# showlab/EgoVLP

Measured on NVIDIA H100. Metric: clips/sec, 16-frame TimeSformer-B + DistilBERT + EgoNCE training step, higher is better.
Workload: dtype bf16

## Files before the change

egovlp_b200/csrc/attention.cu:

```cuda
#include <stdlib.h>

#include "common.cuh"
#include "egovlp_b200.h"

namespace egovlp {

bool space_attn_wgmma_supported(int N);
int space_attn_fwd_wgmma(const void* qkv, void* out, float* lse, float* cls_part, int B, int T, int N, int H,
                         cudaStream_t st);

namespace {

constexpr int HD = 64;
constexpr int ROW_BYTES = 128;
constexpr float LOG2E = 1.4426950408889634f;

struct Geom {
  int B, H, T, N, S, D;
  int mode;
  int PG;
  int G;
  int NP;
  int NPAD;
  int gsize;
};

__device__ __forceinline__ int row_token(const Geom& G, int g, int r) {
  if (r == G.NP) return 0;
  if (r > G.NP) return -1;
  if (G.mode == 1) return 1 + g * G.N + r;
  const int j = r / G.T, f = r - j * G.T, n = g * G.PG + j;
  return n < G.N ? 1 + f * G.N + n : -1;
}

template <int RT>
__device__ __forceinline__ int row_token_x(const Geom& G, int g, int r, int sh) {
  if (RT == 0) return row_token(G, g, r);
  if (r == G.NP) return 0;
  if (r > G.NP) return -1;
  if (RT == 1) return 1 + g * G.N + r;
  const int n = g * G.PG + (r >> sh);
  return n < G.N ? 1 + (r & ((1 << sh) - 1)) * G.N + n : -1;
}

struct Smem {
  uint32_t q, k, v, dout;
  short* gid;
  float* lse;
  float* delta;
  uint32_t stage;
  uint32_t bar;
};

__device__ __forceinline__ bool pair_valid(int gq, int gk, bool first_group) {
  if (gq >= 0) return gk == gq || gk == -2;
  if (gq == -2) return gk >= 0 || (gk == -2 && first_group);
  return false;
}

__device__ __forceinline__ void tile_window(const Geom& G, int r0, int& lo, int& hi) {
  if (r0 <= G.NP && G.NP < r0 + 16) { lo = 0; hi = G.NP; return; }
  if (r0 > G.NP) { lo = 0; hi = 0; return; }
  lo = (r0 / G.gsize) * G.gsize;
  hi = min(G.NP, ((r0 + 15) / G.gsize + 1) * G.gsize);
}
__device__ __forceinline__ bool span_active(const Geom& G, int lo, int hi, int c0, int width) {
  return (c0 < hi && c0 + width > lo) || (c0 <= G.NP && G.NP < c0 + width);
}

template <int RT = 0>
__device__ __forceinline__ void store_rows_bf16(const float (&acc)[8][4], float s0, float s1, uint32_t stage,
                                                uint8_t* stage_gen, bf16* dst, long long ld, int col0, const Geom& G,
                                                int b, int g, int r0, int lane, bool skip_cls, int sh = 0) {
  const int gq = lane >> 2, t = lane & 3;
#pragma unroll
  for (int j = 0; j < 8; ++j) {
    const uint32_t lo = pack_bf16x2(acc[j][0] * s0, acc[j][1] * s0), hi = pack_bf16x2(acc[j][2] * s1, acc[j][3] * s1);
    asm volatile("st.shared.b32 [%0], %1;" ::"r"(sw_addr(stage, gq, j) + t * 4), "r"(lo));
    asm volatile("st.shared.b32 [%0], %1;" ::"r"(sw_addr(stage, gq + 8, j) + t * 4), "r"(hi));
  }
  __syncwarp();
#pragma unroll
  for (int p = 0; p < 4; ++p) {
    const int rr = p * 4 + (lane >> 3), c = lane & 7;
    const int tok = row_token_x<RT>(G, g, r0 + rr, sh);
    if (tok > 0 || (tok == 0 && !skip_cls)) {
      const uint4 v = *reinterpret_cast<const uint4*>(stage_gen + (sw_addr(stage, rr, c) - stage));
      *reinterpret_cast<uint4*>(dst + ((long long)b * G.S + tok) * ld + col0 + c * 8) = v;
    }
  }
  __syncwarp();
}
// ... 1012 lines not shown


}
}

using namespace egovlp;

extern "C" long long egovlp_divided_attn_workspace_floats(int B, int T, int N, int H, int mode) {
  Geom G;
  if (make_geom(G, B, T, N, H, mode)) return -1;
  return (long long)B * H * G.G * 4 * 66;
}

extern "C" int egovlp_divided_attn_fwd(const void* qkv, void* out, float* lse, float* cls_part, int B, int T, int N,
                                       int H, int mode, void* stream) {
  EGOVLP_CHECK_ARG(qkv && out && lse && cls_part, "divided_attn_fwd: null pointer");
  EGOVLP_CHECK_ARG(B > 0 && T > 0 && N > 0 && H > 0 && (mode == 0 || mode == 1), "divided_attn_fwd: bad shape");
  Geom G;
  if (make_geom(G, B, T, N, H, mode)) { set_last_error("divided_attn: unsupported geometry T=%d N=%d", T, N); return EGOVLP_ERR_UNSUPPORTED; }
  CUtensorMap tm;
  int rc = make_group_tmap(&tm, qkv, G, 3 * H);
  if (rc) return rc;
  cudaStream_t st = reinterpret_cast<cudaStream_t>(stream);
  const bf16* q = reinterpret_cast<const bf16*>(qkv);
  bf16* o = reinterpret_cast<bf16*>(out);
  const int grid = B * H * G.G;
#define LAUNCH_FWD(KERN, W, ...)                                                                              \
  do {                                                                                                        \
    const size_t smem = attn_smem_bytes(G, false, W, generic || mode == 1);                                   \
    EGOVLP_CHECK_CUDA(cudaFuncSetAttribute(KERN, cudaFuncAttributeMaxDynamicSharedMemorySize, (int)smem));    \
    KERN<<<grid, W * 32, smem, st>>>(tm, q, o, lse, cls_part, G, ##__VA_ARGS__);                              \
  } while (0)
  const bool generic = force_generic() || (mode == 0 && !time_fast_ok(G));
  if (!generic && mode == 1 && space_attn_wgmma_supported(N)) {
    rc = space_attn_fwd_wgmma(qkv, out, lse, cls_part, B, T, N, H, st);
    if (rc) return rc;
  } else if (generic) {
    if (G.NPAD > 128) LAUNCH_FWD((divided_attn_fwd_kernel<7, 2>), 7);
    else LAUNCH_FWD((divided_attn_fwd_kernel<4, 3>), 4);
  } else if (mode == 1) {
    if (G.NPAD > 128) LAUNCH_FWD((fast_attn_fwd_kernel<false, 7, 2>), 7, 0);
    else LAUNCH_FWD((fast_attn_fwd_kernel<false, 4, 3>), 4, 0);
  } else {
    LAUNCH_FWD((fast_attn_fwd_kernel<true, 4, 4>), 4, time_shift(G));
  }
#undef LAUNCH_FWD
  EGOVLP_CHECK_LAUNCH();
  const int BH = B * H;
  const int parts = (!generic && mode == 0) ? 4 : 1;
  cls_merge_kernel<<<(BH + 3) / 4, 128, 0, st>>>(cls_part, o, lse, BH, H, G.G * parts, G.S, G.D);
  EGOVLP_CHECK_LAUNCH();
  return EGOVLP_OK;
}

extern "C" int egovlp_divided_attn_bwd(const void* qkv, const void* out, const void* dout, const float* lse,
                                       void* dqkv, float* dcls_ws, int B, int T, int N, int H, int mode,
                                       float q_scale, void* stream) {
  EGOVLP_CHECK_ARG(qkv && out && dout && lse && dqkv && dcls_ws, "divided_attn_bwd: null pointer");
  EGOVLP_CHECK_ARG(B > 0 && T > 0 && N > 0 && H > 0 && (mode == 0 || mode == 1), "divided_attn_bwd: bad shape");
  Geom G;
  if (make_geom(G, B, T, N, H, mode)) { set_last_error("divided_attn: unsupported geometry T=%d N=%d", T, N); return EGOVLP_ERR_UNSUPPORTED; }
  CUtensorMap tmq, tmd;
  int rc = make_group_tmap(&tmq, qkv, G, 3 * H);
  if (rc) return rc;
  rc = make_group_tmap(&tmd, dout, G, H);
  if (rc) return rc;
  cudaStream_t st = reinterpret_cast<cudaStream_t>(stream);
  EGOVLP_CHECK_CUDA(cudaMemsetAsync(dcls_ws, 0, (size_t)B * H * 3 * HD * sizeof(float), st));
  const bf16* q = reinterpret_cast<const bf16*>(qkv);
  const bf16* o = reinterpret_cast<const bf16*>(out);
  const bf16* d_o = reinterpret_cast<const bf16*>(dout);
  bf16* dq = reinterpret_cast<bf16*>(dqkv);
  const int grid = B * H * G.G;
#define LAUNCH_BWD(KERN, W, ...)                                                                              \
  do {                                                                                                        \
    const size_t smem = attn_smem_bytes(G, true, W);                                                          \
    EGOVLP_CHECK_CUDA(cudaFuncSetAttribute(KERN, cudaFuncAttributeMaxDynamicSharedMemorySize, (int)smem));    \
    KERN<<<grid, W * 32, smem, st>>>(tmq, tmd, q, o, d_o, lse, dq, dcls_ws, q_scale, G, ##__VA_ARGS__);       \
  } while (0)
  const bool generic = force_generic() || (mode == 0 && !time_fast_ok(G));
  if (generic) {
    if (G.NPAD > 128) LAUNCH_BWD((divided_attn_bwd_kernel<7, 2>), 7);
    else LAUNCH_BWD((divided_attn_bwd_kernel<4, 3>), 4);
  } else if (mode == 1) {
    if (G.NPAD > 128) LAUNCH_BWD((fast_attn_bwd_kernel<false, 7, 2>), 7, 0);
    else LAUNCH_BWD((fast_attn_bwd_kernel<false, 4, 3>), 4, 0);
  } else {
    const char* we = getenv("EGOVLP_ATTN_TIME_BWD_WARPS");
    const bool w8 = we && we[0] == '8';
    if (w8) LAUNCH_BWD((fast_attn_bwd_kernel<true, 8, 2>), 8, time_shift(G));
    else LAUNCH_BWD((fast_attn_bwd_kernel<true, 4, 3>), 4, time_shift(G));
  }
#undef LAUNCH_BWD
  EGOVLP_CHECK_LAUNCH();
  const int n = B * H * 3 * HD;
  cls_grad_finalize_kernel<<<(n + 255) / 256, 256, 0, st>>>(dcls_ws, reinterpret_cast<bf16*>(dqkv), B, H, G.S, G.D, q_scale);
  EGOVLP_CHECK_LAUNCH();
  return EGOVLP_OK;
}
```

egovlp_b200/csrc/attention_wgmma.cu:

```cuda
#include <stdlib.h>

#include "common.cuh"
#include "egovlp_b200.h"

namespace egovlp {
namespace {

constexpr int HD = 64;
constexpr int ROWB = 128;
constexpr int QROWS = 256;
constexpr int KROWS = 208;
constexpr int Q_BYTES = QROWS * ROWB, KV_BYTES = KROWS * ROWB;
constexpr int SMEM_BYTES = Q_BYTES + 2 * KV_BYTES + 1024  + 64 ;
constexpr float LOG2E = 1.4426950408889634f;

struct SpaceGeom {
  int H, T, N, S, D;
};

__device__ __forceinline__ void wgmma_m64n208k16_ss(float (&d)[104], uint64_t adesc, uint64_t bdesc, int scale_d) {
  asm volatile(
      "{\n\t.reg .pred p;\n\t"
      "setp.ne.b32 p, %106, 0;\n\t"
      "wgmma.mma_async.sync.aligned.m64n208k16.f32.bf16.bf16 "
      "{%0,%1,%2,%3,%4,%5,%6,%7,%8,%9,%10,%11,%12,%13,%14,%15,%16,%17,%18,%19,%20,%21,%22,%23,%24,%25,%26,%27,%28,%29,%30,%31,"
      "%32,%33,%34,%35,%36,%37,%38,%39,%40,%41,%42,%43,%44,%45,%46,%47,%48,%49,%50,%51,%52,%53,%54,%55,%56,%57,%58,%59,%60,%61,%62,%63,"
      "%64,%65,%66,%67,%68,%69,%70,%71,%72,%73,%74,%75,%76,%77,%78,%79,%80,%81,%82,%83,%84,%85,%86,%87,%88,%89,%90,%91,%92,%93,%94,%95,"
      "%96,%97,%98,%99,%100,%101,%102,%103}, "
      "%104, %105, p, 1, 1, 0, 0;\n\t}"
      : "+f"(d[0]), "+f"(d[1]), "+f"(d[2]), "+f"(d[3]), "+f"(d[4]), "+f"(d[5]), "+f"(d[6]), "+f"(d[7]),
        "+f"(d[8]), "+f"(d[9]), "+f"(d[10]), "+f"(d[11]), "+f"(d[12]), "+f"(d[13]), "+f"(d[14]), "+f"(d[15]),
        "+f"(d[16]), "+f"(d[17]), "+f"(d[18]), "+f"(d[19]), "+f"(d[20]), "+f"(d[21]), "+f"(d[22]), "+f"(d[23]),
        "+f"(d[24]), "+f"(d[25]), "+f"(d[26]), "+f"(d[27]), "+f"(d[28]), "+f"(d[29]), "+f"(d[30]), "+f"(d[31]),
        "+f"(d[32]), "+f"(d[33]), "+f"(d[34]), "+f"(d[35]), "+f"(d[36]), "+f"(d[37]), "+f"(d[38]), "+f"(d[39]),
        "+f"(d[40]), "+f"(d[41]), "+f"(d[42]), "+f"(d[43]), "+f"(d[44]), "+f"(d[45]), "+f"(d[46]), "+f"(d[47]),
        "+f"(d[48]), "+f"(d[49]), "+f"(d[50]), "+f"(d[51]), "+f"(d[52]), "+f"(d[53]), "+f"(d[54]), "+f"(d[55]),
        "+f"(d[56]), "+f"(d[57]), "+f"(d[58]), "+f"(d[59]), "+f"(d[60]), "+f"(d[61]), "+f"(d[62]), "+f"(d[63]),
        "+f"(d[64]), "+f"(d[65]), "+f"(d[66]), "+f"(d[67]), "+f"(d[68]), "+f"(d[69]), "+f"(d[70]), "+f"(d[71]),
        "+f"(d[72]), "+f"(d[73]), "+f"(d[74]), "+f"(d[75]), "+f"(d[76]), "+f"(d[77]), "+f"(d[78]), "+f"(d[79]),
        "+f"(d[80]), "+f"(d[81]), "+f"(d[82]), "+f"(d[83]), "+f"(d[84]), "+f"(d[85]), "+f"(d[86]), "+f"(d[87]),
        "+f"(d[88]), "+f"(d[89]), "+f"(d[90]), "+f"(d[91]), "+f"(d[92]), "+f"(d[93]), "+f"(d[94]), "+f"(d[95]),
        "+f"(d[96]), "+f"(d[97]), "+f"(d[98]), "+f"(d[99]), "+f"(d[100]), "+f"(d[101]), "+f"(d[102]), "+f"(d[103])
      : "l"(adesc), "l"(bdesc), "r"(scale_d));
}
__device__ __forceinline__ void wgmma_m64n64k16_rs(float (&d)[32], uint32_t a0, uint32_t a1, uint32_t a2, uint32_t a3,
                                                  uint64_t bdesc, int scale_d) {
  asm volatile(
      "{\n\t.reg .pred p;\n\t"
      "setp.ne.b32 p, %37, 0;\n\t"
      "wgmma.mma_async.sync.aligned.m64n64k16.f32.bf16.bf16 "
      "{%0,%1,%2,%3,%4,%5,%6,%7,%8,%9,%10,%11,%12,%13,%14,%15,%16,%17,%18,%19,%20,%21,%22,%23,%24,%25,%26,%27,%28,%29,%30,%31}, "
      "{%32, %33, %34, %35}, %36, p, 1, 1, 1;\n\t}"
      : "+f"(d[0]), "+f"(d[1]), "+f"(d[2]), "+f"(d[3]), "+f"(d[4]), "+f"(d[5]), "+f"(d[6]), "+f"(d[7]),
        "+f"(d[8]), "+f"(d[9]), "+f"(d[10]), "+f"(d[11]), "+f"(d[12]), "+f"(d[13]), "+f"(d[14]), "+f"(d[15]),
        "+f"(d[16]), "+f"(d[17]), "+f"(d[18]), "+f"(d[19]), "+f"(d[20]), "+f"(d[21]), "+f"(d[22]), "+f"(d[23]),
        "+f"(d[24]), "+f"(d[25]), "+f"(d[26]), "+f"(d[27]), "+f"(d[28]), "+f"(d[29]), "+f"(d[30]), "+f"(d[31])
      : "r"(a0), "r"(a1), "r"(a2), "r"(a3), "l"(bdesc), "r"(scale_d));
}

__global__ void __launch_bounds__(256, 1)
space_attn_fwd_wgmma_kernel(const __grid_constant__ CUtensorMap tm_rows, const __grid_constant__ CUtensorMap tm_cls,
                            bf16* __restrict__ out, float* __restrict__ lse_out, float* __restrict__ cls_part, SpaceGeom G) {
  extern __shared__ uint8_t smem_raw[];
  const uint32_t base = (smem_u32(smem_raw) + 1023u) & ~1023u;
  uint8_t* gen = smem_raw + (base - smem_u32(smem_raw));
  const uint32_t sQ = base, sK = base + Q_BYTES, sV = sK + KV_BYTES, bar = sV + KV_BYTES;
  const int g = blockIdx.x;
  const int f = g % G.T, h = (g / G.T) % G.H, b = g / (G.T * G.H);
  const int NK = G.N + 1;

  for (int i = threadIdx.x; i < (Q_BYTES + 2 * KV_BYTES) / 16; i += blockDim.x)
    *reinterpret_cast<uint4*>(gen + 16 * i) = make_uint4(0, 0, 0, 0);
  fence_proxy_async_smem();
  if (threadIdx.x == 0) {
    mbar_init(bar, 1);
    fence_mbar_init();
  }
  __syncthreads();
  if (threadIdx.x == 0) {
    mbar_expect_tx(bar, 3u * (uint32_t)NK * ROWB);
#pragma unroll
    for (int w = 0; w < 3; ++w) {
      const uint32_t dst = w == 0 ? sQ : (w == 1 ? sK : sV);
      tma_load_4d(dst, &tm_rows, bar, 0, 1 + f * G.N, w * G.H + h, b);
      tma_load_4d(dst + G.N * ROWB, &tm_cls, bar, 0, 0, w * G.H + h, b);
    }
  }
  mbar_wait_nocall(bar, 0);

  const int wg = threadIdx.x >> 7, wq = (threadIdx.x >> 5) & 3, lane = threadIdx.x & 31;
  const int gq = lane >> 2, c = lane & 3;
  for (int t = wg; t < QROWS / 64; t += 2) {
    if (t * 64 > G.N) break;
    float s[KROWS / 2];
    wgmma_fence_regs(s);
    wgmma_fence();
#pragma unroll
    for (int kk = 0; kk < HD / 16; ++kk)
      wgmma_m64n208k16_ss(s, make_smem_desc_sw128(sQ + t * 64 * ROWB + kk * 32, 16, 1024),
                          make_smem_desc_sw128(sK + kk * 32, 16, 1024), kk > 0);
    wgmma_commit();
    wgmma_wait<0>();
    wgmma_fence_regs(s);
    const int r0 = t * 64 + wq * 16 + gq;
    float mx[2], sum[2];
#pragma unroll
    for (int h2 = 0; h2 < 2; ++h2) {
      const int vis = (r0 + 8 * h2 == G.N && f != 0) ? G.N : NK;
      float m = -INFINITY;
#pragma unroll
      for (int j = 0; j < KROWS / 8; ++j)
#pragma unroll
        for (int e = 0; e < 2; ++e) {
          float& v = s[4 * j + 2 * h2 + e];
          if (8 * j + 2 * c + e >= vis) v = -INFINITY;
          m = fmaxf(m, v);
        }
      m = fmaxf(m, __shfl_xor_sync(0xffffffffu, m, 1));
      mx[h2] = fmaxf(m, __shfl_xor_sync(0xffffffffu, m, 2));
    }
    uint32_t p[KROWS / 4];
#pragma unroll
    for (int h2 = 0; h2 < 2; ++h2) {
      const float nms = -mx[h2] * LOG2E;
      float acc = 0.f;
#pragma unroll
      for (int j = 0; j < KROWS / 8; ++j) {
        const float e0 = exp2f(fmaf(s[4 * j + 2 * h2], LOG2E, nms));
        const float e1 = exp2f(fmaf(s[4 * j + 2 * h2 + 1], LOG2E, nms));
        acc += e0 + e1;
        p[2 * j + h2] = pack_bf16x2(e0, e1);
      }
      acc += __shfl_xor_sync(0xffffffffu, acc, 1);
      sum[h2] = acc + __shfl_xor_sync(0xffffffffu, acc, 2);
    }
    float o[HD / 2];
    wgmma_fence_regs(o);
    wgmma_fence();
#pragma unroll
    for (int kk = 0; kk < KROWS / 16; ++kk)
      wgmma_m64n64k16_rs(o, p[4 * kk], p[4 * kk + 1], p[4 * kk + 2], p[4 * kk + 3],
                         make_smem_desc_sw128(sV + kk * 16 * ROWB, 8192, 1024), kk > 0);
    wgmma_commit();
    wgmma_wait<0>();
    wgmma_fence_regs(o);
#pragma unroll
    for (int h2 = 0; h2 < 2; ++h2) {
      const int row = r0 + 8 * h2;
      if (row < G.N) {
        const float inv = 1.f / sum[h2];
        const long long tok = (long long)b * G.S + 1 + f * G.N + row;
        bf16* dst = out + tok * G.D + h * HD + 2 * c;
#pragma unroll
        for (int j = 0; j < HD / 8; ++j)
          *reinterpret_cast<uint32_t*>(dst + 8 * j) = pack_bf16x2(o[4 * j + 2 * h2] * inv, o[4 * j + 2 * h2 + 1] * inv);
        if (c == 0) lse_out[((long long)(b * G.H + h)) * G.S + 1 + f * G.N + row] = mx[h2] + logf(sum[h2]);
      } else if (row == G.N) {
        float* dst = cls_part + (((long long)(b * G.H + h)) * G.T + f) * 66;
#pragma unroll
        for (int j = 0; j < HD / 8; ++j) {
          dst[8 * j + 2 * c] = o[4 * j + 2 * h2];
          dst[8 * j + 2 * c + 1] = o[4 * j + 2 * h2 + 1];
        }
        if (c == 0) { dst[64] = mx[h2]; dst[65] = sum[h2]; }
      }
    }
  }
}

}

bool space_attn_wgmma_supported(int N) {
  const char* e = getenv("EGOVLP_ATTN_TC");
  if (!(e && e[0] == '1')) return false;
  return N + 1 > 128 && N + 1 <= KROWS;
}

int space_attn_fwd_wgmma(const void* qkv, void* out, float* lse, float* cls_part, int B, int T, int N, int H,
                         cudaStream_t st) {
  SpaceGeom G;
  G.H = H; G.T = T; G.N = N; G.S = 1 + T * N; G.D = H * HD;
  const uint64_t W = 3ull * G.D;
  const uint64_t dims[4] = {HD, (uint64_t)G.S, (uint64_t)(3 * H), (uint64_t)B};
  const uint64_t strides[4] = {1, W, HD, (uint64_t)G.S * W};
  const uint32_t box_rows[4] = {HD, (uint32_t)N, 1, 1};
  const uint32_t box_cls[4] = {HD, 1, 1, 1};
  CUtensorMap tm_rows, tm_cls;
  int rc = make_tmap_nd_bf16(&tm_rows, qkv, 4, dims, strides, box_rows, true);
  if (rc) return rc;
  rc = make_tmap_nd_bf16(&tm_cls, qkv, 4, dims, strides, box_cls, true);
  if (rc) return rc;
  static bool attr = false;
  if (!attr) {
    EGOVLP_CHECK_CUDA(cudaFuncSetAttribute(space_attn_fwd_wgmma_kernel, cudaFuncAttributeMaxDynamicSharedMemorySize,
                                           SMEM_BYTES));
    attr = true;
  }
  space_attn_fwd_wgmma_kernel<<<B * H * T, 256, SMEM_BYTES, st>>>(tm_rows, tm_cls, reinterpret_cast<bf16*>(out), lse,
                                                                   cls_part, G);
  EGOVLP_CHECK_LAUNCH();
  return EGOVLP_OK;
}

}
```

Baseline: 185.6.

## Add wgmma tensor-core backward kernel for space attention

Adds a Hopper wgmma-based backward kernel for divided space attention (one block per batch/head/frame). It TMA-loads Q, K, V and dO into swizzled shared memory and computes delta in-kernel. It then computes S^T and dP^T per 64-row key tile with wgmma, forms P and dS in registers for the dV/dK register-sourced MMAs, and stages dS in smem for a second dQ pass. It is enabled by default for space mode whenever N+1 is in range, replacing the mma.sync fast kernel. The cost is heavy smem use (one block per SM) and atomics for CLS gradients.

```diff
diff --git a/egovlp_b200/csrc/attention.cu b/egovlp_b200/csrc/attention.cu
--- a/egovlp_b200/csrc/attention.cu
+++ b/egovlp_b200/csrc/attention.cu
@@ -8,6 +8,9 @@
 bool space_attn_wgmma_supported(int N);
 int space_attn_fwd_wgmma(const void* qkv, void* out, float* lse, float* cls_part, int B, int T, int N, int H,
                          cudaStream_t st);
+bool space_attn_bwd_wgmma_supported(int N);
+int space_attn_bwd_wgmma(const void* qkv, const void* out, const void* dout, const float* lse, void* dqkv, float* dcls,
+                         float q_scale, int B, int T, int N, int H, cudaStream_t st);
 
 namespace {
 
@@ -1186,6 +1189,9 @@
   if (generic) {
     if (G.NPAD > 128) LAUNCH_BWD((divided_attn_bwd_kernel<7, 2>), 7);
     else LAUNCH_BWD((divided_attn_bwd_kernel<4, 3>), 4);
+  } else if (mode == 1 && space_attn_bwd_wgmma_supported(N)) {
+    rc = space_attn_bwd_wgmma(qkv, out, dout, lse, dqkv, dcls_ws, q_scale, B, T, N, H, st);
+    if (rc) return rc;
   } else if (mode == 1) {
     if (G.NPAD > 128) LAUNCH_BWD((fast_attn_bwd_kernel<false, 7, 2>), 7, 0);
     else LAUNCH_BWD((fast_attn_bwd_kernel<false, 4, 3>), 4, 0);
diff --git a/egovlp_b200/csrc/attention_wgmma.cu b/egovlp_b200/csrc/attention_wgmma.cu
--- a/egovlp_b200/csrc/attention_wgmma.cu
+++ b/egovlp_b200/csrc/attention_wgmma.cu
@@ -58,6 +58,37 @@
       : "r"(a0), "r"(a1), "r"(a2), "r"(a3), "l"(bdesc), "r"(scale_d));
 }
 
+__device__ __forceinline__ void wgmma_m64n112k16_ss(float (&d)[56], uint64_t adesc, uint64_t bdesc, int scale_d) {
+  asm volatile(
+      "{\n\t.reg .pred p;\n\t"
+      "setp.ne.b32 p, %58, 0;\n\t"
+      "wgmma.mma_async.sync.aligned.m64n112k16.f32.bf16.bf16 "
+      "{%0,%1,%2,%3,%4,%5,%6,%7,%8,%9,%10,%11,%12,%13,%14,%15,%16,%17,%18,%19,%20,%21,%22,%23,%24,%25,%26,%27,%28,%29,%30,%31,"
+      "%32,%33,%34,%35,%36,%37,%38,%39,%40,%41,%42,%43,%44,%45,%46,%47,%48,%49,%50,%51,%52,%53,%54,%55}, "
+      "%56, %57, p, 1, 1, 0, 0;\n\t}"
+      : "+f"(d[0]), "+f"(d[1]), "+f"(d[2]), "+f"(d[3]), "+f"(d[4]), "+f"(d[5]), "+f"(d[6]), "+f"(d[7]),
+        "+f"(d[8]), "+f"(d[9]), "+f"(d[10]), "+f"(d[11]), "+f"(d[12]), "+f"(d[13]), "+f"(d[14]), "+f"(d[15]),
+        "+f"(d[16]), "+f"(d[17]), "+f"(d[18]), "+f"(d[19]), "+f"(d[20]), "+f"(d[21]), "+f"(d[22]), "+f"(d[23]),
+        "+f"(d[24]), "+f"(d[25]), "+f"(d[26]), "+f"(d[27]), "+f"(d[28]), "+f"(d[29]), "+f"(d[30]), "+f"(d[31]),
+        "+f"(d[32]), "+f"(d[33]), "+f"(d[34]), "+f"(d[35]), "+f"(d[36]), "+f"(d[37]), "+f"(d[38]), "+f"(d[39]),
+        "+f"(d[40]), "+f"(d[41]), "+f"(d[42]), "+f"(d[43]), "+f"(d[44]), "+f"(d[45]), "+f"(d[46]), "+f"(d[47]),
+        "+f"(d[48]), "+f"(d[49]), "+f"(d[50]), "+f"(d[51]), "+f"(d[52]), "+f"(d[53]), "+f"(d[54]), "+f"(d[55])
+      : "l"(adesc), "l"(bdesc), "r"(scale_d));
+}
+__device__ __forceinline__ void wgmma_m64n64k16_ss_tt(float (&d)[32], uint64_t adesc, uint64_t bdesc, int scale_d) {
+  asm volatile(
+      "{\n\t.reg .pred p;\n\t"
+      "setp.ne.b32 p, %34, 0;\n\t"
+      "wgmma.mma_async.sync.aligned.m64n64k16.f32.bf16.bf16 "
+      "{%0,%1,%2,%3,%4,%5,%6,%7,%8,%9,%10,%11,%12,%13,%14,%15,%16,%17,%18,%19,%20,%21,%22,%23,%24,%25,%26,%27,%28,%29,%30,%31}, "
+      "%32, %33, p, 1, 1, 1, 1;\n\t}"
+      : "+f"(d[0]), "+f"(d[1]), "+f"(d[2]), "+f"(d[3]), "+f"(d[4]), "+f"(d[5]), "+f"(d[6]), "+f"(d[7]),
+        "+f"(d[8]), "+f"(d[9]), "+f"(d[10]), "+f"(d[11]), "+f"(d[12]), "+f"(d[13]), "+f"(d[14]), "+f"(d[15]),
+        "+f"(d[16]), "+f"(d[17]), "+f"(d[18]), "+f"(d[19]), "+f"(d[20]), "+f"(d[21]), "+f"(d[22]), "+f"(d[23]),
+        "+f"(d[24]), "+f"(d[25]), "+f"(d[26]), "+f"(d[27]), "+f"(d[28]), "+f"(d[29]), "+f"(d[30]), "+f"(d[31])
+      : "l"(adesc), "l"(bdesc), "r"(scale_d));
+}
+
 __global__ void __launch_bounds__(256, 1)
 space_attn_fwd_wgmma_kernel(const __grid_constant__ CUtensorMap tm_rows, const __grid_constant__ CUtensorMap tm_cls,
                             bf16* __restrict__ out, float* __restrict__ lse_out, float* __restrict__ cls_part, SpaceGeom G) {
@@ -168,27 +199,276 @@
   }
 }
 
+constexpr int BQC = 112;
+constexpr int BQROWS = 2 * BQC;
+constexpr int DS_SLAB = KROWS * ROWB;
+constexpr int B_V = KV_BYTES, B_Q = 2 * KV_BYTES, B_DO = B_Q + BQROWS * ROWB, B_DS = B_DO + BQROWS * ROWB;
+constexpr int B_LSE = B_DS + 4 * DS_SLAB, B_DELTA = B_LSE + BQROWS * 4, B_BAR = B_DELTA + BQROWS * 4;
+constexpr int BWD_SMEM_BYTES = B_BAR + 8 + 1024 ;
+static_assert(BWD_SMEM_BYTES <= 232448, "space attention backward: dynamic smem over the sm_90 limit");
+
+template <bool MASK>
+__device__ __forceinline__ void p_ds_fragments(const float (&st)[BQC / 2], const float (&dpt)[BQC / 2],
+                                               uint32_t (&pf)[BQC / 4], uint32_t (&dsf)[BQC / 4],
+                                               const float* s_lse, const float* s_delta, uint32_t sDS, int q0, int kr0,
+                                               int NP, bool first_group) {
+#pragma unroll
+  for (int j = 0; j < BQC / 8; ++j) {
+    const int q = q0 + 8 * j;
+    const float2 ls = *reinterpret_cast<const float2*>(s_lse + q);
+    const float2 de = *reinterpret_cast<const float2*>(s_delta + q);
+#pragma unroll
+    for (int h2 = 0; h2 < 2; ++h2) {
+      const int kr = kr0 + 8 * h2;
+      bool v0 = true, v1 = true;
+      if (MASK) {
+        const bool kpatch = kr < NP, kcls = kr == NP;
+        v0 = q <= NP && (kpatch || (kcls && (q < NP || first_group)));
+        v1 = q + 1 <= NP && (kpatch || (kcls && (q + 1 < NP || first_group)));
+      }
+      const float p0 = v0 ? exp2f(fmaf(st[4 * j + 2 * h2], LOG2E, -ls.x)) : 0.f;
+      const float p1 = v1 ? exp2f(fmaf(st[4 * j + 2 * h2 + 1], LOG2E, -ls.y)) : 0.f;
+      const float d0 = v0 ? p0 * (dpt[4 * j + 2 * h2] - de.x) : 0.f;
+      const float d1 = v1 ? p1 * (dpt[4 * j + 2 * h2 + 1] - de.y) : 0.f;
+      pf[2 * j + h2] = pack_bf16x2(p0, p1);
+      dsf[2 * j + h2] = pack_bf16x2(d0, d1);
+      if (!MASK || kr < KROWS)
+        asm volatile("st.shared.b32 [%0], %1;" ::"r"(sDS + (q >> 6) * DS_SLAB + kr * ROWB +
+                                                     ((((q & 63) >> 3) ^ (kr & 7)) << 4) + (q & 7) * 2),
+                     "r"(dsf[2 * j + h2]));
+    }
+  }
+}
+
+__global__ void __launch_bounds__(256, 1)
+space_attn_bwd_wgmma_kernel(const __grid_constant__ CUtensorMap tm_rows, const __grid_constant__ CUtensorMap tm_cls,
+                            const __grid_constant__ CUtensorMap tm_do_rows,
+                            const __grid_constant__ CUtensorMap tm_do_cls, const bf16* __restrict__ out,
+                            const float* __restrict__ lse_in, bf16* __restrict__ dqkv, float* __restrict__ dcls,
+                            float q_scale, SpaceGeom G) {
+  extern __shared__ uint8_t smem_raw[];
+  const uint32_t base = (smem_u32(smem_raw) + 1023u) & ~1023u;
+  uint8_t* gen = smem_raw + (base - smem_u32(smem_raw));
+  const uint32_t sK = base, sV = base + B_V, sQ = base + B_Q, sdO = base + B_DO, sDS = base + B_DS, bar = base + B_BAR;
+  float* s_lse = reinterpret_cast<float*>(gen + B_LSE);
+  float* s_delta = reinterpret_cast<float*>(gen + B_DELTA);
+  const int h = blockIdx.x % G.H, f = (blockIdx.x / G.H) % G.T, b = blockIdx.x / (G.H * G.T);
+  const int NP = G.N, NK = G.N + 1, tid = threadIdx.x;
+  const long long tok0 = (long long)b * G.S + 1 + (long long)f * G.N;
+
+  for (int i = tid; i < (BQROWS - NK) * 8; i += blockDim.x) {
+    const int r = NK + (i >> 3), o = r * ROWB + (i & 7) * 16;
+    const uint4 z = make_uint4(0, 0, 0, 0);
+    *reinterpret_cast<uint4*>(gen + B_Q + o) = z;
+    *reinterpret_cast<uint4*>(gen + B_DO + o) = z;
+    if (r < KROWS) {
+      *reinterpret_cast<uint4*>(gen + o) = z;
+      *reinterpret_cast<uint4*>(gen + B_V + o) = z;
+    }
+  }
+  for (int i = tid + ((NK + 63) / 64) * 64 * 8; i < KROWS * 8; i += blockDim.x)
+#pragma unroll
+    for (int s = 0; s < 4; ++s) *reinterpret_cast<uint4*>(gen + B_DS + s * DS_SLAB + i * 16) = make_uint4(0, 0, 0, 0);
+  fence_proxy_async_smem();
+  if (tid == 0) {
+    mbar_init(bar, 1);
+    fence_mbar_init();
+  }
+  __syncthreads();
+  if (tid == 0) {
+    mbar_expect_tx(bar, 4u * (uint32_t)NK * ROWB);
+#pragma unroll
+    for (int w = 0; w < 3; ++w) {
+      const uint32_t dst = w == 0 ? sQ : (w == 1 ? sK : sV);
+      tma_load_4d(dst, &tm_rows, bar, 0, 1 + f * G.N, w * G.H + h, b);
+      tma_load_4d(dst + NP * ROWB, &tm_cls, bar, 0, 0, w * G.H + h, b);
+    }
+    tma_load_4d(sdO, &tm_do_rows, bar, 0, 1 + f * G.N, h, b);
+    tma_load_4d(sdO + NP * ROWB, &tm_do_cls, bar, 0, 0, h, b);
+  }
+
+  constexpr int PR = BQROWS / 32;
+  uint4 o_pre[PR];
+  float l_pre[PR];
+#pragma unroll
+  for (int i = 0; i < PR; ++i) {
+    const int r = (tid >> 3) + 32 * i;
+    const long long tok = r < NP ? tok0 + r : (long long)b * G.S;
+    o_pre[i] = __ldg(reinterpret_cast<const uint4*>(out + tok * G.D + h * HD + (tid & 7) * 8));
+    l_pre[i] = __ldg(lse_in + (long long)(b * G.H + h) * G.S + (tok - (long long)b * G.S));
+  }
+  mbar_wait_nocall(bar, 0);
+#pragma unroll
+  for (int i = 0; i < PR; ++i) {
+    const int r = (tid >> 3) + 32 * i, cc = tid & 7;
+    const uint4 dv = *reinterpret_cast<const uint4*>(gen + (sw_addr(sdO, r, cc) - base));
+    const uint32_t ou[4] = {o_pre[i].x, o_pre[i].y, o_pre[i].z, o_pre[i].w}, du[4] = {dv.x, dv.y, dv.z, dv.w};
+    float d = 0.f;
+#pragma unroll
+    for (int k = 0; k < 4; ++k) {
+      const float2 a = unpack_bf16x2(ou[k]), bb = unpack_bf16x2(du[k]);
+      d += a.x * bb.x + a.y * bb.y;
+    }
+    d += __shfl_xor_sync(0xffffffffu, d, 1);
+    d += __shfl_xor_sync(0xffffffffu, d, 2);
+    d += __shfl_xor_sync(0xffffffffu, d, 4);
+    if (cc == 0) {
+      s_delta[r] = r <= NP ? d : 0.f;
+      s_lse[r] = r <= NP ? l_pre[i] * LOG2E : 0.f;
+    }
+  }
+  __syncthreads();
+
+  const int wg = tid >> 7, wq = (tid >> 5) & 3, lane = tid & 31;
+  const int gq = lane >> 2, c = lane & 3;
+  const int ntiles = (NK + 63) / 64;
+  const bool first_group = f == 0;
+  const long long ld = 3LL * G.D;
+  float* dcls_bh = dcls + (long long)(b * G.H + h) * 3 * HD;
+
+  for (int kt = wg; kt < ntiles; kt += 2) {
+    const int kr0 = kt * 64 + wq * 16 + gq;
+    float dk[HD / 2], dv[HD / 2];
+#pragma unroll 1
+    for (int qc = 0; qc < 2; ++qc) {
+      float st[BQC / 2], dpt[BQC / 2];
+      wgmma_fence_regs(st);
+      wgmma_fence_regs(dpt);
+      wgmma_fence();
+#pragma unroll
+      for (int kk = 0; kk < HD / 16; ++kk)
+        wgmma_m64n112k16_ss(st, make_smem_desc_sw128(sK + kt * 64 * ROWB + kk * 32, 16, 1024),
+                            make_smem_desc_sw128(sQ + qc * BQC * ROWB + kk * 32, 16, 1024), kk > 0);
+#pragma unroll
+      for (int kk = 0; kk < HD / 16; ++kk)
+        wgmma_m64n112k16_ss(dpt, make_smem_desc_sw128(sV + kt * 64 * ROWB + kk * 32, 16, 1024),
+                            make_smem_desc_sw128(sdO + qc * BQC * ROWB + kk * 32, 16, 1024), kk > 0);
+      wgmma_commit();
+      wgmma_wait<0>();
+      wgmma_fence_regs(st);
+      wgmma_fence_regs(dpt);
+      uint32_t pf[BQC / 4], dsf[BQC / 4];
+      if (kt * 64 + 64 <= NP && qc * BQC + BQC <= NP)
+        p_ds_fragments<false>(st, dpt, pf, dsf, s_lse, s_delta, sDS, qc * BQC + 2 * c, kr0, NP, first_group);
+      else
+        p_ds_fragments<true>(st, dpt, pf, dsf, s_lse, s_delta, sDS, qc * BQC + 2 * c, kr0, NP, first_group);
+      wgmma_fence_regs(dk);
+      wgmma_fence_regs(dv);
+      wgmma_fence();
+#pragma unroll
+      for (int kk = 0; kk < BQC / 16; ++kk)
+        wgmma_m64n64k16_rs(dv, pf[4 * kk], pf[4 * kk + 1], pf[4 * kk + 2], pf[4 * kk + 3],
+                           make_smem_desc_sw128(sdO + (qc * BQC + kk * 16) * ROWB, 8192, 1024), qc > 0 || kk > 0);
+#pragma unroll
+      for (int kk = 0; kk < BQC / 16; ++kk)
+        wgmma_m64n64k16_rs(dk, dsf[4 * kk], dsf[4 * kk + 1], dsf[4 * kk + 2], dsf[4 * kk + 3],
+                           make_smem_desc_sw128(sQ + (qc * BQC + kk * 16) * ROWB, 8192, 1024), qc > 0 || kk > 0);
+      wgmma_commit();
+      wgmma_wait<0>();
+      wgmma_fence_regs(dk);
+      wgmma_fence_regs(dv);
+    }
+#pragma unroll
+    for (int h2 = 0; h2 < 2; ++h2) {
+      const int kr = kr0 + 8 * h2;
+      if (kr < NP) {
+        bf16* pk = dqkv + (tok0 + kr) * ld + G.D + h * HD + 2 * c;
+#pragma unroll
+        for (int j = 0; j < HD / 8; ++j) {
+          *reinterpret_cast<uint32_t*>(pk + 8 * j) = pack_bf16x2(dk[4 * j + 2 * h2], dk[4 * j + 2 * h2 + 1]);
+          *reinterpret_cast<uint32_t*>(pk + G.D + 8 * j) = pack_bf16x2(dv[4 * j + 2 * h2], dv[4 * j + 2 * h2 + 1]);
+        }
+      } else if (kr == NP) {
+#pragma unroll
+        for (int j = 0; j < HD / 8; ++j)
+#pragma unroll
+          for (int e = 0; e < 2; ++e) {
+            atomicAdd(dcls_bh + HD + 8 * j + 2 * c + e, dk[4 * j + 2 * h2 + e]);
+            atomicAdd(dcls_bh + 2 * HD + 8 * j + 2 * c + e, dv[4 * j + 2 * h2 + e]);
+          }
+      }
+    }
+  }
+  fence_proxy_async_smem();
+  __syncthreads();
+
+  for (int qt = wg; qt < ntiles; qt += 2) {
+    float dq[HD / 2];
+    wgmma_fence_regs(dq);
+    wgmma_fence();
+#pragma unroll
+    for (int kk = 0; kk < KROWS / 16; ++kk)
+      wgmma_m64n64k16_ss_tt(dq, make_smem_desc_sw128(sDS + qt * DS_SLAB + kk * 16 * ROWB, DS_SLAB, 1024),
+                              make_smem_desc_sw128(sK + kk * 16 * ROWB, 8192, 1024), kk > 0);
+    wgmma_commit();
+    wgmma_wait<0>();
+    wgmma_fence_regs(dq);
+#pragma unroll
+    for (int h2 = 0; h2 < 2; ++h2) {
+      const int r = qt * 64 + wq * 16 + gq + 8 * h2;
+      if (r < NP) {
+        bf16* pq = dqkv + (tok0 + r) * ld + h * HD + 2 * c;
+#pragma unroll
+        for (int j = 0; j < HD / 8; ++j)
+          *reinterpret_cast<uint32_t*>(pq + 8 * j) =
+              pack_bf16x2(dq[4 * j + 2 * h2] * q_scale, dq[4 * j + 2 * h2 + 1] * q_scale);
+      } else if (r == NP) {
+#pragma unroll
+        for (int j = 0; j < HD / 8; ++j) {
+          atomicAdd(dcls_bh + 8 * j + 2 * c, dq[4 * j + 2 * h2]);
+          atomicAdd(dcls_bh + 8 * j + 2 * c + 1, dq[4 * j + 2 * h2 + 1]);
+        }
+      }
+    }
+  }
+}
+
+int make_row_maps(CUtensorMap* rows, CUtensorMap* cls, const void* base, int ncolblk, int B, int S, int N) {
+  const uint64_t W = (uint64_t)ncolblk * HD;
+  const uint64_t dims[4] = {HD, (uint64_t)S, (uint64_t)ncolblk, (uint64_t)B};
+  const uint64_t strides[4] = {1, W, HD, (uint64_t)S * W};
+  const uint32_t box_rows[4] = {HD, (uint32_t)N, 1, 1};
+  const uint32_t box_cls[4] = {HD, 1, 1, 1};
+  int rc = make_tmap_nd_bf16(rows, base, 4, dims, strides, box_rows, true);
+  if (rc) return rc;
+  return make_tmap_nd_bf16(cls, base, 4, dims, strides, box_cls, true);
+}
+
+bool space_attn_wgmma_range(int N) { return N + 1 > 128 && N + 1 <= KROWS; }
+
 }
 
 bool space_attn_wgmma_supported(int N) {
   const char* e = getenv("EGOVLP_ATTN_TC");
   if (!(e && e[0] == '1')) return false;
-  return N + 1 > 128 && N + 1 <= KROWS;
+  return space_attn_wgmma_range(N);
+}
+bool space_attn_bwd_wgmma_supported(int N) { return space_attn_wgmma_range(N); }
+
+int space_attn_bwd_wgmma(const void* qkv, const void* out, const void* dout, const float* lse, void* dqkv, float* dcls,
+                         float q_scale, int B, int T, int N, int H, cudaStream_t st) {
+  SpaceGeom G;
+  G.H = H; G.T = T; G.N = N; G.S = 1 + T * N; G.D = H * HD;
+  CUtensorMap tm_rows, tm_cls, tm_do_rows, tm_do_cls;
+  int rc = make_row_maps(&tm_rows, &tm_cls, qkv, 3 * H, B, G.S, N);
+  if (rc) return rc;
+  rc = make_row_maps(&tm_do_rows, &tm_do_cls, dout, H, B, G.S, N);
+  if (rc) return rc;
+  EGOVLP_CHECK_CUDA(cudaFuncSetAttribute(space_attn_bwd_wgmma_kernel, cudaFuncAttributeMaxDynamicSharedMemorySize,
+                                         BWD_SMEM_BYTES));
+  space_attn_bwd_wgmma_kernel<<<B * H * T, 256, BWD_SMEM_BYTES, st>>>(
+      tm_rows, tm_cls, tm_do_rows, tm_do_cls, reinterpret_cast<const bf16*>(out), lse, reinterpret_cast<bf16*>(dqkv),
+      dcls, q_scale, G);
+  EGOVLP_CHECK_LAUNCH();
+  return EGOVLP_OK;
 }
 
 int space_attn_fwd_wgmma(const void* qkv, void* out, float* lse, float* cls_part, int B, int T, int N, int H,
                          cudaStream_t st) {
   SpaceGeom G;
   G.H = H; G.T = T; G.N = N; G.S = 1 + T * N; G.D = H * HD;
-  const uint64_t W = 3ull * G.D;
-  const uint64_t dims[4] = {HD, (uint64_t)G.S, (uint64_t)(3 * H), (uint64_t)B};
-  const uint64_t strides[4] = {1, W, HD, (uint64_t)G.S * W};
-  const uint32_t box_rows[4] = {HD, (uint32_t)N, 1, 1};
-  const uint32_t box_cls[4] = {HD, 1, 1, 1};
   CUtensorMap tm_rows, tm_cls;
-  int rc = make_tmap_nd_bf16(&tm_rows, qkv, 4, dims, strides, box_rows, true);
-  if (rc) return rc;
-  rc = make_tmap_nd_bf16(&tm_cls, qkv, 4, dims, strides, box_cls, true);
+  int rc = make_row_maps(&tm_rows, &tm_cls, qkv, 3 * H, B, G.S, N);
   if (rc) return rc;
   static bool attr = false;
   if (!attr) {
```

Result: faster. 187.7, median of 6 (+1.1%).

## Add WGMMA-based space-attention backward kernel with TMA loads

Applied to the files above, without the earlier changes.

Adds a Hopper wgmma backward kernel for divided space attention. Each CTA handles one (batch, head, frame) block and loads Q, K, V and dO into swizzled shared memory via TMA. It recomputes the probabilities from the saved LSE and computes dQ, dK and dV with m64n208 and m64n64 wgmma instructions. It is selected by default when N+1 falls between 129 and 208, replacing the mma.sync fast backward path. The CLS-token gradients are accumulated with float atomics. The shared-memory footprint is large, and it recomputes S once in the dQ pass and again in the dK/dV pass.

```diff
diff --git a/egovlp_b200/csrc/attention.cu b/egovlp_b200/csrc/attention.cu
--- a/egovlp_b200/csrc/attention.cu
+++ b/egovlp_b200/csrc/attention.cu
@@ -8,6 +8,9 @@
 bool space_attn_wgmma_supported(int N);
 int space_attn_fwd_wgmma(const void* qkv, void* out, float* lse, float* cls_part, int B, int T, int N, int H,
                          cudaStream_t st);
+bool space_attn_bwd_wgmma_selected(int N);
+int space_attn_bwd_wgmma(const void* qkv, const void* out, const void* dout, const float* lse, void* dqkv, float* dcls,
+                         int B, int T, int N, int H, float q_scale, cudaStream_t st);
 
 namespace {
 
@@ -1187,7 +1190,10 @@
     if (G.NPAD > 128) LAUNCH_BWD((divided_attn_bwd_kernel<7, 2>), 7);
     else LAUNCH_BWD((divided_attn_bwd_kernel<4, 3>), 4);
   } else if (mode == 1) {
-    if (G.NPAD > 128) LAUNCH_BWD((fast_attn_bwd_kernel<false, 7, 2>), 7, 0);
+    if (space_attn_bwd_wgmma_selected(N)) {
+      rc = space_attn_bwd_wgmma(qkv, out, dout, lse, dqkv, dcls_ws, B, T, N, H, q_scale, st);
+      if (rc) return rc;
+    } else if (G.NPAD > 128) LAUNCH_BWD((fast_attn_bwd_kernel<false, 7, 2>), 7, 0);
     else LAUNCH_BWD((fast_attn_bwd_kernel<false, 4, 3>), 4, 0);
   } else {
     const char* we = getenv("EGOVLP_ATTN_TIME_BWD_WARPS");
diff --git a/egovlp_b200/csrc/attention_wgmma.cu b/egovlp_b200/csrc/attention_wgmma.cu
--- a/egovlp_b200/csrc/attention_wgmma.cu
+++ b/egovlp_b200/csrc/attention_wgmma.cu
@@ -1,4 +1,5 @@
 #include <stdlib.h>
+#include <string.h>
 
 #include "common.cuh"
 #include "egovlp_b200.h"
@@ -168,6 +169,241 @@
   }
 }
 
+constexpr int BWD_SMEM_BYTES = 4 * KV_BYTES + 2 * KROWS * 4 + 16  + 1024 ;
+
+__device__ __forceinline__ int bwd_tile_row0(int t) { return t < 3 ? 64 * t : KROWS - 64; }
+
+__device__ __forceinline__ void bwd_store_rows(const float (&o)[HD / 2], float scale, int r0, int first, bf16* dqkv,
+                                               float* dcls, int col, const SpaceGeom& G, int b, int f, int c) {
+#pragma unroll
+  for (int h2 = 0; h2 < 2; ++h2) {
+    const int row = r0 + 8 * h2;
+    if (row < first || row > G.N) continue;
+    if (row < G.N) {
+      const long long tok = (long long)b * G.S + 1 + f * G.N + row;
+      bf16* dst = dqkv + tok * 3 * G.D + col + 2 * c;
+#pragma unroll
+      for (int j = 0; j < HD / 8; ++j)
+        *reinterpret_cast<uint32_t*>(dst + 8 * j) = pack_bf16x2(o[4 * j + 2 * h2] * scale, o[4 * j + 2 * h2 + 1] * scale);
+    } else {
+#pragma unroll
+      for (int j = 0; j < HD / 8; ++j) {
+        atomicAdd(dcls + 8 * j + 2 * c, o[4 * j + 2 * h2]);
+        atomicAdd(dcls + 8 * j + 2 * c + 1, o[4 * j + 2 * h2 + 1]);
+      }
+    }
+  }
+}
+
+__global__ void __launch_bounds__(128, 2)
+space_attn_bwd_wgmma_kernel(const __grid_constant__ CUtensorMap tm_rows, const __grid_constant__ CUtensorMap tm_cls,
+                            const __grid_constant__ CUtensorMap tm_do_rows, const __grid_constant__ CUtensorMap tm_do_cls,
+                            const bf16* __restrict__ out, const float* __restrict__ lse_in, bf16* __restrict__ dqkv,
+                            float* __restrict__ dcls, float q_scale, SpaceGeom G) {
+  extern __shared__ uint8_t smem_raw[];
+  const uint32_t base = (smem_u32(smem_raw) + 1023u) & ~1023u;
+  uint8_t* gen = smem_raw + (base - smem_u32(smem_raw));
+  const uint32_t sQ = base, sK = sQ + KV_BYTES, sV = sK + KV_BYTES, sD = sV + KV_BYTES;
+  float* lse_s = reinterpret_cast<float*>(gen + 4 * KV_BYTES);
+  float* delta_s = lse_s + KROWS;
+  const uint32_t bar = base + 4 * KV_BYTES + 2 * KROWS * 4;
+  const int h = blockIdx.x % G.H, f = (blockIdx.x / G.H) % G.T, b = blockIdx.x / (G.H * G.T);
+  const int NK = G.N + 1, tid = threadIdx.x;
+
+  for (int i = tid; i < 4 * (KROWS - NK) * 8; i += 128) {
+    const int w = i / ((KROWS - NK) * 8), r = NK + (i >> 3) % (KROWS - NK);
+    *reinterpret_cast<uint4*>(gen + w * KV_BYTES + r * ROWB + (i & 7) * 16) = make_uint4(0, 0, 0, 0);
+  }
+  fence_proxy_async_smem();
+  if (tid == 0) {
+    mbar_init(bar, 1);
+    fence_mbar_init();
+  }
+  __syncthreads();
+  if (tid == 0) {
+    mbar_expect_tx(bar, 4u * (uint32_t)NK * ROWB);
+#pragma unroll
+    for (int w = 0; w < 3; ++w) {
+      const uint32_t dst = w == 0 ? sQ : (w == 1 ? sK : sV);
+      tma_load_4d(dst, &tm_rows, bar, 0, 1 + f * G.N, w * G.H + h, b);
+      tma_load_4d(dst + G.N * ROWB, &tm_cls, bar, 0, 0, w * G.H + h, b);
+    }
+    tma_load_4d(sD, &tm_do_rows, bar, 0, 1 + f * G.N, h, b);
+    tma_load_4d(sD + G.N * ROWB, &tm_do_cls, bar, 0, 0, h, b);
+  }
+
+  constexpr int PRE = KROWS / 16;
+  const int rr = tid >> 3, cc = tid & 7;
+  uint4 o_pre[PRE];
+  float l_pre[PRE];
+#pragma unroll
+  for (int i = 0; i < PRE; ++i) {
+    const int r = rr + 16 * i;
+    const int tok = r < G.N ? 1 + f * G.N + r : 0;
+    o_pre[i] = __ldg(reinterpret_cast<const uint4*>(out + ((long long)b * G.S + tok) * G.D + h * HD + cc * 8));
+    l_pre[i] = __ldg(lse_in + (long long)(b * G.H + h) * G.S + tok);
+  }
+  mbar_wait_nocall(bar, 0);
+#pragma unroll
+  for (int i = 0; i < PRE; ++i) {
+    const int r = rr + 16 * i;
+    const uint4 dv = *reinterpret_cast<const uint4*>(gen + 3 * KV_BYTES + r * ROWB + ((cc ^ (r & 7)) << 4));
+    const uint32_t ou[4] = {o_pre[i].x, o_pre[i].y, o_pre[i].z, o_pre[i].w}, du[4] = {dv.x, dv.y, dv.z, dv.w};
+    float d = 0.f;
+#pragma unroll
+    for (int k = 0; k < 4; ++k) {
+      const float2 a = unpack_bf16x2(ou[k]), e = unpack_bf16x2(du[k]);
+      d += a.x * e.x + a.y * e.y;
+    }
+    d += __shfl_xor_sync(0xffffffffu, d, 1);
+    d += __shfl_xor_sync(0xffffffffu, d, 2);
+    d += __shfl_xor_sync(0xffffffffu, d, 4);
+    if (cc == 0) {
+      delta_s[r] = r < NK ? d : 0.f;
+      lse_s[r] = r < NK ? l_pre[i] * LOG2E : INFINITY;
+    }
+  }
+  __syncthreads();
+
+  const int wq = tid >> 5, lane = tid & 31, gq = lane >> 2, c = lane & 3;
+  const int cls_hidden = f != 0 ? G.N : -1;
+  float* dcls_g = dcls + (long long)(b * G.H + h) * 3 * HD;
+
+  float dq[HD / 2];
+  int r0_prev = 0;
+  for (int t = 0; t < 4 && 64 * t < NK; ++t) {
+    const int m0 = bwd_tile_row0(t), r0 = m0 + wq * 16 + gq;
+    float s[KROWS / 2];
+    wgmma_fence_regs(s);
+    wgmma_fence();
+#pragma unroll
+    for (int kk = 0; kk < HD / 16; ++kk)
+      wgmma_m64n208k16_ss(s, make_smem_desc_sw128(sQ + m0 * ROWB + kk * 32, 16, 1024),
+                          make_smem_desc_sw128(sK + kk * 32, 16, 1024), kk > 0);
+    wgmma_commit();
+    wgmma_wait<0>();
+    if (t > 0) {
+      wgmma_fence_regs(dq);
+      bwd_store_rows(dq, q_scale, r0_prev, 64 * (t - 1), dqkv, dcls_g, h * HD, G, b, f, c);
+    }
+    wgmma_fence_regs(s);
+    uint32_t p[KROWS / 4];
+#pragma unroll
+    for (int h2 = 0; h2 < 2; ++h2) {
+      const int row = r0 + 8 * h2;
+      const float nl = -lse_s[row];
+      const int lim = (row == G.N && f != 0) ? G.N : NK;
+#pragma unroll
+      for (int j = 0; j < KROWS / 8; ++j) {
+        const int col = 8 * j + 2 * c;
+        const float e0 = (j >= 16 && col >= lim) ? 0.f : exp2f(fmaf(s[4 * j + 2 * h2], LOG2E, nl));
+        const float e1 = (j >= 16 && col + 1 >= lim) ? 0.f : exp2f(fmaf(s[4 * j + 2 * h2 + 1], LOG2E, nl));
+        p[2 * j + h2] = pack_bf16x2(e0, e1);
+      }
+    }
+    wgmma_fence_regs(s);
+    wgmma_fence();
+#pragma unroll
+    for (int kk = 0; kk < HD / 16; ++kk)
+      wgmma_m64n208k16_ss(s, make_smem_desc_sw128(sD + m0 * ROWB + kk * 32, 16, 1024),
+                          make_smem_desc_sw128(sV + kk * 32, 16, 1024), kk > 0);
+    wgmma_commit();
+    wgmma_wait<0>();
+    wgmma_fence_regs(s);
+#pragma unroll
+    for (int h2 = 0; h2 < 2; ++h2) {
+      const float de = delta_s[r0 + 8 * h2];
+#pragma unroll
+      for (int j = 0; j < KROWS / 8; ++j) {
+        const float2 pp = unpack_bf16x2(p[2 * j + h2]);
+        p[2 * j + h2] = pack_bf16x2(pp.x * (s[4 * j + 2 * h2] - de), pp.y * (s[4 * j + 2 * h2 + 1] - de));
+      }
+    }
+    wgmma_fence_regs(dq);
+    wgmma_fence();
+#pragma unroll
+    for (int kk = 0; kk < KROWS / 16; ++kk)
+      wgmma_m64n64k16_rs(dq, p[4 * kk], p[4 * kk + 1], p[4 * kk + 2], p[4 * kk + 3],
+                         make_smem_desc_sw128(sK + kk * 16 * ROWB, 8192, 1024), kk > 0);
+    wgmma_commit();
+    r0_prev = r0;
+  }
+  const int nt = (NK + 63) / 64;
+  wgmma_wait<0>();
+  wgmma_fence_regs(dq);
+  bwd_store_rows(dq, q_scale, r0_prev, 64 * (nt - 1), dqkv, dcls_g, h * HD, G, b, f, c);
+
+  float dk[HD / 2];
+  int k0_prev = 0;
+  for (int t = 0; t < 4 && 64 * t < NK; ++t) {
+    const int m0 = bwd_tile_row0(t), k0 = m0 + wq * 16 + gq;
+    float s[KROWS / 2];
+    wgmma_fence_regs(s);
+    wgmma_fence();
+#pragma unroll
+    for (int kk = 0; kk < HD / 16; ++kk)
+      wgmma_m64n208k16_ss(s, make_smem_desc_sw128(sK + m0 * ROWB + kk * 32, 16, 1024),
+                          make_smem_desc_sw128(sQ + kk * 32, 16, 1024), kk > 0);
+    wgmma_commit();
+    wgmma_wait<0>();
+    if (t > 0) {
+      wgmma_fence_regs(dk);
+      bwd_store_rows(dk, 1.f, k0_prev, 64 * (t - 1), dqkv, dcls_g + HD, G.D + h * HD, G, b, f, c);
+    }
+    wgmma_fence_regs(s);
+    uint32_t p[KROWS / 4];
+#pragma unroll
+    for (int j = 0; j < KROWS / 8; ++j) {
+      const int col = 8 * j + 2 * c;
+      const float2 ls = *reinterpret_cast<const float2*>(lse_s + col);
+#pragma unroll
+      for (int h2 = 0; h2 < 2; ++h2) {
+        const int hid = k0 + 8 * h2 == G.N ? cls_hidden : -1;
+        const float e0 = (j >= 16 && col == hid) ? 0.f : exp2f(fmaf(s[4 * j + 2 * h2], LOG2E, -ls.x));
+        const float e1 = (j >= 16 && col + 1 == hid) ? 0.f : exp2f(fmaf(s[4 * j + 2 * h2 + 1], LOG2E, -ls.y));
+        p[2 * j + h2] = pack_bf16x2(e0, e1);
+      }
+    }
+    float dv[HD / 2];
+    wgmma_fence_regs(dv);
+    wgmma_fence_regs(s);
+    wgmma_fence();
+#pragma unroll
+    for (int kk = 0; kk < KROWS / 16; ++kk)
+      wgmma_m64n64k16_rs(dv, p[4 * kk], p[4 * kk + 1], p[4 * kk + 2], p[4 * kk + 3],
+                         make_smem_desc_sw128(sD + kk * 16 * ROWB, 8192, 1024), kk > 0);
+#pragma unroll
+    for (int kk = 0; kk < HD / 16; ++kk)
+      wgmma_m64n208k16_ss(s, make_smem_desc_sw128(sV + m0 * ROWB + kk * 32, 16, 1024),
+                          make_smem_desc_sw128(sD + kk * 32, 16, 1024), kk > 0);
+    wgmma_commit();
+    wgmma_wait<0>();
+    wgmma_fence_regs(s);
+    wgmma_fence_regs(dv);
+    bwd_store_rows(dv, 1.f, k0, 64 * t, dqkv, dcls_g + 2 * HD, 2 * G.D + h * HD, G, b, f, c);
+#pragma unroll
+    for (int j = 0; j < KROWS / 8; ++j) {
+      const float2 de = *reinterpret_cast<const float2*>(delta_s + 8 * j + 2 * c);
+#pragma unroll
+      for (int h2 = 0; h2 < 2; ++h2) {
+        const float2 pp = unpack_bf16x2(p[2 * j + h2]);
+        p[2 * j + h2] = pack_bf16x2(pp.x * (s[4 * j + 2 * h2] - de.x), pp.y * (s[4 * j + 2 * h2 + 1] - de.y));
+      }
+    }
+    wgmma_fence_regs(dk);
+    wgmma_fence();
+#pragma unroll
+    for (int kk = 0; kk < KROWS / 16; ++kk)
+      wgmma_m64n64k16_rs(dk, p[4 * kk], p[4 * kk + 1], p[4 * kk + 2], p[4 * kk + 3],
+                         make_smem_desc_sw128(sQ + kk * 16 * ROWB, 8192, 1024), kk > 0);
+    wgmma_commit();
+    k0_prev = k0;
+  }
+  wgmma_wait<0>();
+  wgmma_fence_regs(dk);
+  bwd_store_rows(dk, 1.f, k0_prev, 64 * (nt - 1), dqkv, dcls_g + HD, G.D + h * HD, G, b, f, c);
+}
+
 }
 
 bool space_attn_wgmma_supported(int N) {
@@ -202,4 +438,40 @@
   return EGOVLP_OK;
 }
 
-}
+bool space_attn_bwd_wgmma_selected(int N) {
+  const char* e = getenv("EGOVLP_ATTN_SPACE_BWD");
+  if (e && strcmp(e, "mma") == 0) return false;
+  return N + 1 > 128 && N + 1 <= KROWS;
+}
+
+int space_attn_bwd_wgmma(const void* qkv, const void* out, const void* dout, const float* lse, void* dqkv, float* dcls,
+                         int B, int T, int N, int H, float q_scale, cudaStream_t st) {
+  SpaceGeom G;
+  G.H = H; G.T = T; G.N = N; G.S = 1 + T * N; G.D = H * HD;
+  const uint64_t W = 3ull * G.D;
+  const uint64_t dims[4] = {HD, (uint64_t)G.S, (uint64_t)(3 * H), (uint64_t)B};
+  const uint64_t strides[4] = {1, W, HD, (uint64_t)G.S * W};
+  const uint64_t dims_do[4] = {HD, (uint64_t)G.S, (uint64_t)H, (uint64_t)B};
+  const uint64_t strides_do[4] = {1, (uint64_t)G.D, HD, (uint64_t)G.S * G.D};
+  const uint32_t box_rows[4] = {HD, (uint32_t)N, 1, 1};
+  const uint32_t box_cls[4] = {HD, 1, 1, 1};
+  CUtensorMap tm_rows, tm_cls, tm_do_rows, tm_do_cls;
+  int rc = make_tmap_nd_bf16(&tm_rows, qkv, 4, dims, strides, box_rows, true);
+  if (!rc) rc = make_tmap_nd_bf16(&tm_cls, qkv, 4, dims, strides, box_cls, true);
+  if (!rc) rc = make_tmap_nd_bf16(&tm_do_rows, dout, 4, dims_do, strides_do, box_rows, true);
+  if (!rc) rc = make_tmap_nd_bf16(&tm_do_cls, dout, 4, dims_do, strides_do, box_cls, true);
+  if (rc) return rc;
+  static bool attr = false;
+  if (!attr) {
+    EGOVLP_CHECK_CUDA(cudaFuncSetAttribute(space_attn_bwd_wgmma_kernel, cudaFuncAttributeMaxDynamicSharedMemorySize,
+                                           BWD_SMEM_BYTES));
+    attr = true;
+  }
+  space_attn_bwd_wgmma_kernel<<<B * H * T, 128, BWD_SMEM_BYTES, st>>>(
+      tm_rows, tm_cls, tm_do_rows, tm_do_cls, reinterpret_cast<const bf16*>(out), lse, reinterpret_cast<bf16*>(dqkv),
+      dcls, q_scale, G);
+  EGOVLP_CHECK_LAUNCH();
+  return EGOVLP_OK;
+}
+
+}
```

After: 180.4 before, 183.6 after, median of 6. 1.02x the previous value.
